# dusk-network/plonk

Measured on AMD Instinct MI355X. Metric: prove() wall-clock (ms) at 2^20 gates, lower is better.
Workload: dtype u32 limbs (Fr 256-bit / Fp 384-bit Montgomery)

## Files before the change

### plonk_amd/csrc/capi.hip

```cpp
#include <chrono>
#include <cstdio>
#include <cstring>
#include <sched.h>
#include <thread>

#include "plonk_internal.hpp"
#include "hostg1.hpp"

namespace plonk {

static thread_local char g_last_error[512] = "";

void set_last_error(const char* what, const char* detail, const char* file, int line) {
  snprintf(g_last_error, sizeof g_last_error, "%s:%d: %s -> %s", file, line, what ? what : "?", detail ? detail : "?");
}

int srs_generate_device(Ctx* c, const Fr& tau, const Fr& g_scalar, uint64_t n, G1Affine* out_dev);

int ctx_refuse_poisoned(const char* api_fn) {
  set_last_error(api_fn, "context unusable: a collective timed out and its stream never drained (comm_sync); destroy the context", __FILE__, __LINE__);
  return PLONK_ERR_STATE;
}

bool ctx_abandon(Ctx* c) {
  if (!c->comm_poisoned) return false;
  const auto t0 = std::chrono::steady_clock::now();
  for (;;) {
    const bool busy = (c->main_stream && hipStreamQuery(c->main_stream) == hipErrorNotReady) ||
                      (c->side_stream && hipStreamQuery(c->side_stream) == hipErrorNotReady);
    if (!busy) return false;
    if (std::chrono::duration_cast<std::chrono::milliseconds>(std::chrono::steady_clock::now() - t0).count() > 2000) return true;
    std::this_thread::sleep_for(std::chrono::microseconds(500));
  }
}

void xyzz_to_affine97_host(const G1& p, uint8_t out[97]) {
  G1Affine a;
  const bool finite = p.to_affine(&a);
  memcpy(out, a.x.l, 48);
  memcpy(out + 48, a.y.l, 48);
  out[96] = finite ? 0 : 1;
}

struct ProfRec { int slot; hipEvent_t a, b; };
struct ProfState {
  std::vector<hipEvent_t> pool;
  size_t used = 0;
  std::vector<ProfRec> recs;
  hipEvent_t open[Ctx::PROF_SLOTS] = {nullptr};
};
static std::map<Ctx*, ProfState*> g_prof;
static std::mutex g_prof_mu;

static ProfState* prof_state(Ctx* c) {
  std::lock_guard<std::mutex> lk(g_prof_mu);
  auto it = g_prof.find(c);
  if (it != g_prof.end()) return it->second;
  return g_prof[c] = new ProfState();
}
static void prof_release(Ctx* c) {
  ProfState* ps = nullptr;
  {
    std::lock_guard<std::mutex> lk(g_prof_mu);
    auto it = g_prof.find(c);
    if (it == g_prof.end()) return;
    ps = it->second;
    g_prof.erase(it);
  }
  for (hipEvent_t e : ps->pool) (void)hipEventDestroy(e);
  delete ps;
}
static void prof_forget(Ctx* c) {
  std::lock_guard<std::mutex> lk(g_prof_mu);
  auto it = g_prof.find(c);
  if (it != g_prof.end()) { delete it->second; g_prof.erase(it); }
}
static hipEvent_t prof_event(ProfState* ps) {
  if (ps->used == ps->pool.size()) {
    hipEvent_t e;
    if (hipEventCreate(&e) != hipSuccess) return nullptr;
    ps->pool.push_back(e);
  }
  return ps->pool[ps->used++];
}
void prof_begin(Ctx* c, int slot) {
  if (!c->profile) return;
  ProfState* ps = prof_state(c);
  hipEvent_t e = prof_event(ps);
  if (!e) return;
  (void)hipEventRecord(e, c->stream);
  ps->open[slot] = e;
}
void prof_end(Ctx* c, int slot) {
  if (!c->profile) return;
  ProfState* ps = prof_state(c);
  if (!ps->open[slot]) return;
  hipEvent_t e = prof_event(ps);
  if (!e) return;
  (void)hipEventRecord(e, c->stream);
  ps->recs.push_back({slot, ps->open[slot], e});
  ps->open[slot] = nullptr;
}
void prof_host_add(Ctx* c, int slot, double ms) {
  if (!c->profile) return;
  c->acc_ms[slot] += ms;
  c->acc_n[slot] += 1;
}
static int prof_collect(Ctx* c) {
  ProfState* ps = prof_state(c);
  HIP_TRY(hipStreamSynchronize(c->stream));
  for (auto& r : ps->recs) {
    float ms = 0;
    if (hipEventElapsedTime(&ms, r.a, r.b) == hipSuccess) {
      c->acc_ms[r.slot] += ms;
      c->acc_n[r.slot] += 1;
    }
  }
  ps->recs.clear();
  ps->used = 0;
  return PLONK_OK;
}

static int ensure_ntt_staging(Ctx* c, uint64_t n) {
  if (n <= c->ntt_cap) return PLONK_OK;
  if (c->ntt_buf) {
    HIP_TRY(hipStreamSynchronize(c->stream));
    HIP_TRY(hipFree(c->ntt_buf)); HIP_TRY(hipFree(c->ntt_buf2)); HIP_TRY(hipFree(c->ntt_buf3)); HIP_TRY(hipFree(c->ntt_tmp));
    c->ntt_buf = c->ntt_buf2 = c->ntt_buf3 = c->ntt_tmp = nullptr; c->ntt_cap = 0;
  }
  HIP_TRY(hipMalloc((void**)&c->ntt_buf, sizeof(Fr) * n));
  HIP_TRY(hipMalloc((void**)&c->ntt_buf2, sizeof(Fr) * n));
  HIP_TRY(hipMalloc((void**)&c->ntt_buf3, sizeof(Fr) * n));
  HIP_TRY(hipMalloc((void**)&c->ntt_tmp, sizeof(Fr) * n));
  c->ntt_cap = n;
  return PLONK_OK;
}

int msm_group_sums(Ctx* c, const Fr* const* scalars_dev, const uint64_t* m, int cnt, G1* sums) {
  G1* res[MSM_MAX_BATCH];
  for (int k = 0; k < cnt; ++k) res[k] = (G1*)c->msm.result + (size_t)k * MSM_BIT_SUMS;
  const int rc = msm_batch_device(c, scalars_dev, m, cnt, res, true);
  if (rc) return rc;
  HIP_TRY(hipMemcpyAsync(c->msm.result_host, c->msm.result, sizeof(G1) * MSM_BIT_SUMS * cnt, hipMemcpyDeviceToHost, c->stream));
  HIP_TRY(hipStreamSynchronize(c->stream));
  for (int k = 0; k < cnt; ++k)
    sums[k] = finish_bit_sums(reinterpret_cast<const G1*>(c->msm.result_host) + (size_t)k * MSM_BIT_SUMS, c->msm.last_rowbits,
                              c->srs_rows == MSM_ROWS_BITPOS);
  return PLONK_OK;
}

static int ensure_scalar_staging(Ctx* c, uint64_t m) {
  MsmWork& w = c->msm;
  if (m <= w.cap_stage) return PLONK_OK;
  if (w.scalars_stage) { HIP_TRY(hipFree(w.scalars_stage)); w.scalars_stage = nullptr; w.cap_stage = 0; }
  HIP_TRY(hipMalloc((void**)&w.scalars_stage, sizeof(Fr) * m));
  w.cap_stage = m;
  return PLONK_OK;
}

}

using namespace plonk;

namespace plonk {

static int env_int(const char* name, int dflt) { const char* e = getenv(name); return e && e[0] ? atoi(e) : dflt; }
static char env_chr(const char* name) { const char* e = getenv(name); return e ? e[0] : 0; }

void config_resolve(const plonk_gpu_config* user, int device, Config* out) {
  Config g;
  plonk_gpu_config u{};
  if (user) memcpy(&u, user, user->struct_size < sizeof(u) ? user->struct_size : sizeof(u));
  g.table_budget = u.table_budget_bytes;
  g.table_mode = u.table_mode;
  g.bucket_bits = u.msm_bucket_bits;
  g.quotient_domain = u.quotient_domain == 8 ? 8 : 4;
  g.wire_commit_coeff = u.wire_commit == 1;
  g.shard_quotient = u.shard_quotient;
  g.shard_z = u.shard_grand_product;
  g.shard_side = u.shard_side_stream;
  g.ntt_elog = u.ntt_elements_log2;
  g.comm_timeout_ms = u.comm_timeout_ms > 0 ? u.comm_timeout_ms : 120000;
  g.side_cus = u.side_stream_cus;
  switch (env_chr("PLONK_MSM_TABLE")) { case 'w': g.table_mode = MSM_ROWS_WINDOW; break; case 'h': g.table_mode = MSM_ROWS_HALFPOS; break; case 'b': g.table_mode = MSM_ROWS_BITPOS; break; default: break; }
  if (const int mb = env_int("PLONK_TABLE_BUDGET_MB", 0); mb > 0) g.table_budget = (uint64_t)mb << 20;
  if (const int b = env_int("PLONK_MSM_BUCKETS", 0); b) g.bucket_bits = b;
  if (env_chr("PLONK_QUOTIENT_DOMAIN") == '8') g.quotient_domain = 8;
  if (env_chr("PLONK_QUOTIENT_DOMAIN") == '4') g.quotient_domain = 4;
  if (env_chr("PLONK_WIRE_COMMIT") == 'c') g.wire_commit_coeff = 1;
  if (env_chr("PLONK_Z_COMMIT") == 'c') g.z_commit_coeff = 1;
  if (env_chr("PLONK_Z_COMMIT") == 'e') g.z_commit_coeff = -1;
  if (const char v = env_chr("PLONK_SHARD_QUOTIENT")) g.shard_quotient = v == '0' ? -1 : 1;
  if (const char v = env_chr("PLONK_SHARD_Z")) g.shard_z = v == '1' ? 1 : -1;
  if (const char v = env_chr("PLONK_SHARD_SIDE")) g.shard_side = v == '0' ? -1 : 1;
  if (const char v = env_chr("PLONK_NTT_ELOG"); v == '2' || v == '3') g.ntt_elog = v - '0';
  if (const int t = env_int("PLONK_COMM_TIMEOUT_MS", 0); t > 0) g.comm_timeout_ms = t;
  if (getenv("PLONK_SIDE_CUS")) g.side_cus = env_int("PLONK_SIDE_CUS", 0);
  g.ksl = env_int("PLONK_MSM_KSL", 0);
  g.prof_fine = env_chr("PLONK_PROF_FINE") == '1';
  g.acc_lds = env_chr("PLONK_MSM_ACC") == 'l';
  if (const char v = env_chr("PLONK_MSM_ORDER")) g.order = v == '1' ? 1 : 0;
  g.tail_serial = env_chr("PLONK_MSM_TAIL") == 's';
  g.bsum_lane = env_chr("PLONK_MSM_BSUM") == 'l';
  g.rc_lane_tree = env_chr("PLONK_MSM_RCTREE") == 'l';
  g.lps = env_int("PLONK_MSM_LPS", 0);
  g.rcwv = env_int("PLONK_MSM_RCWV", 0);
  if (const char v = env_chr("PLONK_MSM_SORT13")) g.sort13 = v == '1' ? 1 : 0;
  g.acc_wg = env_int("PLONK_MSM_ACC_WG", 0);
  g.ntt_direct = env_chr("PLONK_NTT_DIRECT") != '0';
  g.bi_cfg = env_int("PLONK_BI_CFG", -1);
  if (const char v = env_chr("PLONK_SIDE_DEFER")) g.side_defer = v == '1' ? 1 : (v == '2' ? 2 : 0);
  if (const char v = env_chr("PLONK_SIDE_AFTER_ELOG"); v == '2' || v == '3') g.side_after_elog = v - '0';
  if (const char v = env_chr("PLONK_WIRE_POLYS_SIDE")) g.wire_polys_side = v == '1' ? 1 : 0;
  if (env_chr("PLONK_WIRE_BY_COLUMN") == '0') g.wire_by_column = -1;
  if (env_chr("PLONK_WIRE_BY_COLUMN") == '1') g.wire_by_column = 1;
  if (env_chr("PLONK_WIRE_BY_COLUMN") == '2') g.wire_by_column = 2;
  if (getenv("PLONK_HOST_THREADS")) g.host_threads = env_int("PLONK_HOST_THREADS", -1);
  if (g.table_mode != (int)MSM_ROWS_WINDOW && g.table_mode != (int)MSM_ROWS_HALFPOS && g.table_mode != (int)MSM_ROWS_BITPOS) g.table_mode = 0;
  if (g.ntt_elog != 2 && g.ntt_elog != 3) g.ntt_elog = 0;
  if (g.side_cus < 0) g.side_cus = 0;
  if (g.host_threads < 0) {
    cpu_set_t set;
    CPU_ZERO(&set);
    const int cpus = sched_getaffinity(0, sizeof set, &set) == 0 ? CPU_COUNT(&set) : (int)std::thread::hardware_concurrency();
    g.host_threads = cpus >= 8 ? 3 : 0;
  }
  if (g.host_threads > 7) g.host_threads = 7;
  if (g.table_budget == 0) {
    size_t total = 0;
    if (hipDeviceTotalMem(&total, device) != hipSuccess || total == 0) total = 256ull << 30;
    g.table_budget = (uint64_t)total / 10 * 8;
  }
  *out = g;
}

static int config_check(const plonk_gpu_config* u, const char* api_fn) {
  if (!u) return PLONK_OK;
  if (u->struct_size < 8 || u->struct_size > 4096) return (set_last_error("invalid argument", "plonk_gpu_config.struct_size is not set", __FILE__, __LINE__), PLONK_ERR_ARG);
  plonk_gpu_config c{};
  memcpy(&c, u, u->struct_size < sizeof(c) ? u->struct_size : sizeof(c));
  auto bad = [&](const char* what) { set_last_error(api_fn, what, __FILE__, __LINE__); return PLONK_ERR_ARG; };
  if (c.table_mode != PLONK_TABLE_AUTO && c.table_mode != PLONK_TABLE_WINDOW && c.table_mode != PLONK_TABLE_HALFPOS && c.table_mode != PLONK_TABLE_BITPOS) return bad("plonk_gpu_config.table_mode");
  if (c.msm_bucket_bits != 0 && c.msm_bucket_bits != 15 && c.msm_bucket_bits != 17 && c.msm_bucket_bits != 19) return bad("plonk_gpu_config.msm_bucket_bits");
  if (c.quotient_domain != 0 && c.quotient_domain != 4 && c.quotient_domain != 8) return bad("plonk_gpu_config.quotient_domain");
  if (c.wire_commit != 0 && c.wire_commit != 1) return bad("plonk_gpu_config.wire_commit");
  if (c.ntt_elements_log2 != 0 && c.ntt_elements_log2 != 2 && c.ntt_elements_log2 != 3) return bad("plonk_gpu_config.ntt_elements_log2");
  for (int v : {c.shard_quotient, c.shard_grand_product, c.shard_side_stream}) if (v < -1 || v > 1) return bad("plonk_gpu_config.shard_*: -1, 0 or 1");
  if (c.comm_timeout_ms < 0 || c.side_stream_cus < -1 || c.side_stream_cus > 200) return bad("plonk_gpu_config.comm_timeout_ms / side_stream_cus");
  return PLONK_OK;
}

static int side_stream_partition(Ctx* c) {
  const int k = c->cfg.side_cus;
  if (k <= 0) return PLONK_OK;
  hipDeviceProp_t prop;
  HIP_TRY(hipGetDeviceProperties(&prop, c->device));
  const int ncu = prop.multiProcessorCount;
  if (k >= ncu) return (set_last_error("plonk_gpu_config.side_stream_cus", "must be smaller than the device's compute-unit count", __FILE__, __LINE__), PLONK_ERR_ARG);
  const int words = (ncu + 31) / 32;
  std::vector<uint32_t> side(words, 0u);
  for (int i = 0; i < ncu; ++i)
    if ((int64_t)i * k / ncu != (int64_t)(i + 1) * k / ncu) side[i / 32] |= 1u << (i % 32);
  hipStream_t ss = nullptr;
  if (hipExtStreamCreateWithCUMask(&ss, (uint32_t)words, side.data()) != hipSuccess) return (set_last_error("hipExtStreamCreateWithCUMask", "side stream", __FILE__, __LINE__), PLONK_ERR_HIP);
  (void)hipStreamDestroy(c->side_stream);
  c->side_stream = ss;
  return PLONK_OK;
}

}

extern "C" {

const char* plonk_last_error(void) { return g_last_error; }

static int create_context(plonk_ctx** out, int dev, const plonk_gpu_config* config, const char* api_fn) {
  if (!out) return PLONK_ERR_ARG;
  { const int rc = config_check(config, api_fn); if (rc) return rc; }
  int count = 0;
  if (hipGetDeviceCount(&count) != hipSuccess || count == 0) {
    set_last_error("hipGetDeviceCount", "no HIP device visible", __FILE__, __LINE__);
    return PLONK_ERR_NO_GPU;
  }
  if (dev < 0 || dev >= count) return PLONK_ERR_ARG;
  HIP_TRY(hipSetDevice(dev));
  auto* ctx = new plonk_ctx();
  ctx->c.device = dev;
  config_resolve(config, dev, &ctx->c.cfg);
  int prio_least = 0, prio_greatest = 0;
  (void)hipDeviceGetStreamPriorityRange(&prio_least, &prio_greatest);
  hipError_t e = hipStreamCreateWithPriority(&ctx->c.stream, hipStreamNonBlocking, prio_greatest);
  if (e == hipSuccess) e = hipStreamCreateWithPriority(&ctx->c.side_stream, hipStreamNonBlocking, prio_least);
  ctx->c.main_stream = ctx->c.stream;
  if (e != hipSuccess) {
    set_last_error("hipStreamCreate", hipGetErrorString(e), __FILE__, __LINE__);
    delete ctx;
    return PLONK_ERR_HIP;
  }
  { const int rc = side_stream_partition(&ctx->c); if (rc) { (void)hipStreamDestroy(ctx->c.stream); (void)hipStreamDestroy(ctx->c.side_stream); delete ctx; return rc; } }
  *out = ctx;
  return PLONK_OK;
}

int plonk_ctx_create(plonk_ctx** out, const int* devices, int ndev) {
  const char* const api_fn = __func__;
  return plonk::api_guard(api_fn, [&]() -> int {
  if (!out || ndev > 1 || ndev < 0) return PLONK_ERR_ARG;
  return create_context(out, (devices && ndev == 1) ? devices[0] : 0, nullptr, api_fn);
  });
}

int plonk_ctx_create_ex(plonk_ctx** out, int device, const plonk_gpu_config* config) {
  const char* const api_fn = __func__;
  return plonk::api_guard(api_fn, [&]() -> int { return create_context(out, device, config, api_fn); });
}

int plonk_ctx_get_config(plonk_ctx* ctx, plonk_gpu_config* out) {
  const char* const api_fn = __func__;
  return plonk::api_guard(api_fn, [&]() -> int {
  if (!ctx || !out || out->struct_size < 8 || out->struct_size > 4096) return (set_last_error("invalid argument", "plonk_ctx_get_config: set struct_size = sizeof(plonk_gpu_config)", __FILE__, __LINE__), PLONK_ERR_ARG);
  std::lock_guard<std::mutex> lk(ctx->c.mu);
  const Config& g = ctx->c.cfg;
  plonk_gpu_config full{};
  full.struct_size = (uint32_t)sizeof(plonk_gpu_config);
  full.table_budget_bytes = g.table_budget;
  full.table_mode = g.table_mode;
  full.msm_bucket_bits = g.bucket_bits;
  full.quotient_domain = g.quotient_domain;
  full.wire_commit = g.wire_commit_coeff;
  full.shard_quotient = g.shard_quotient;
  full.shard_grand_product = g.shard_z;
  full.shard_side_stream = g.shard_side;
  full.ntt_elements_log2 = g.ntt_elog;
  full.comm_timeout_ms = g.comm_timeout_ms;
  full.side_stream_cus = g.side_cus;
  const uint32_t want = out->struct_size < sizeof(full) ? out->struct_size : (uint32_t)sizeof(full);
  memcpy(out, &full, want);
  out->struct_size = want;
  return PLONK_OK;
  });
}

int plonk_ctx_set_config(plonk_ctx* ctx, const plonk_gpu_config* config) {
  const char* const api_fn = __func__;
  return plonk::api_guard(api_fn, [&]() -> int {
  if (!ctx) return PLONK_ERR_ARG;
  { const int rc = config_check(config, api_fn); if (rc) return rc; }
  std::lock_guard<std::mutex> lk(ctx->c.mu);
  Config next;
  config_resolve(config, ctx->c.device, &next);
  if (next.side_cus != ctx->c.cfg.side_cus)
    return (set_last_error("plonk_ctx_set_config", "side_stream_cus can only be chosen at plonk_ctx_create_ex", __FILE__, __LINE__), PLONK_ERR_STATE);
  ctx->c.cfg = next;
  return PLONK_OK;
  });
}

int plonk_ctx_table_bytes(plonk_ctx* ctx, uint64_t* in_use, uint64_t* budget) {
  const char* const api_fn = __func__;
  return plonk::api_guard(api_fn, [&]() -> int {
  if (!ctx) return PLONK_ERR_ARG;
  std::lock_guard<std::mutex> lk(ctx->c.mu);
  if (in_use) *in_use = ctx->c.table_bytes;
  if (budget) *budget = ctx->c.cfg.table_budget;
  return PLONK_OK;
  });
}

static void plan_out(const plonk_msm_plan_internal& p, plonk_msm_plan* out) {
  memset(out, 0, sizeof(*out));
  out->table_rows = p.table_rows; out->bucket_bits = p.bucket_bits; out->digit_width = p.digit_width;
  out->slice_entries = p.slice_entries; out->ordered_lanes = p.ordered_lanes; out->wide_words = p.wide_words; out->flags = p.flags; out->terms = p.terms;
  snprintf(out->accumulate_kernel, sizeof(out->accumulate_kernel), "%s", p.kernel);
}

int plonk_ctx_describe_msm(plonk_ctx* ctx, uint64_t m, int count, int bit_sum_tail, uint32_t table_rows, uint64_t table_points, plonk_msm_plan* out) {
  const char* const api_fn = __func__;
  return plonk::api_guard(api_fn, [&]() -> int {
  if (!ctx || !out || count < 1 || count > MSM_MAX_BATCH) return PLONK_ERR_ARG;
  std::lock_guard<std::mutex> lk(ctx->c.mu);
  Ctx& c = ctx->c;
  if (table_rows == 0) { table_rows = c.srs_rows; table_points = c.srs_n; if (!c.srs_table) return PLONK_ERR_NO_SRS; }
  if (table_rows != MSM_ROWS_WINDOW && table_rows != MSM_ROWS_HALFPOS && table_rows != MSM_ROWS_BITPOS) return PLONK_ERR_ARG;
  plonk_msm_plan_internal p;
  msm_plan(&c, table_rows, table_points, m, count, bit_sum_tail != 0, &p);
  plan_out(p, out);
  return PLONK_OK;
  });
}

int plonk_ctx_last_msm(plonk_ctx* ctx, plonk_msm_plan* out) {
  const char* const api_fn = __func__;
  return plonk::api_guard(api_fn, [&]() -> int {
  if (!ctx || !out) return PLONK_ERR_ARG;
  std::lock_guard<std::mutex> lk(ctx->c.mu);
  if (!ctx->c.last_plan.table_rows) return (set_last_error("plonk_ctx_last_msm", "no MSM has run on this context", __FILE__, __LINE__), PLONK_ERR_STATE);
  plan_out(ctx->c.last_plan, out);
  return PLONK_OK;
  });
}

void plonk_ctx_destroy(plonk_ctx* ctx) {
  if (!ctx) return;
  (void)plonk_comm_destroy(ctx);
  Ctx& c = ctx->c;
  finish_pool_release(&c);
  (void)hipSetDevice(c.device);
  if (ctx_abandon(&c)) {
    prof_forget(&c);
    delete ctx;
    return;
  }
  (void)hipStreamSynchronize(c.stream);
  verify_ws_release(&c);
  kzg_ws_release(&c);
  for (auto& kv : c.ntt_tables) {
    NttTables* t = kv.second;
    (void)hipFree(t->tw_lo); (void)hipFree(t->tw_hi); (void)hipFree(t->tw_lo_scaled);
    (void)hipFree(t->w512); (void)hipFree(t->g_lo); (void)hipFree(t->g_hi);
    (void)hipFree(t->tw_lo29); (void)hipFree(t->tw_hi29); (void)hipFree(t->tw_lo_scaled29);
    (void)hipFree(t->w512_29); (void)hipFree(t->g_lo29); (void)hipFree(t->g_hi29);
    (void)hipFree(t->tw_a29); (void)hipFree(t->tw_b29);
    delete t;
  }
  (void)hipFree(c.ntt_buf); (void)hipFree(c.ntt_buf2); (void)hipFree(c.ntt_buf3); (void)hipFree(c.ntt_tmp);
  if (c.down_stream) (void)hipStreamDestroy(c.down_stream);
  if (c.copy_stream) (void)hipStreamDestroy(c.copy_stream); (void)hipFree(c.srs_table); (void)hipFree(c.table_scratch);
  MsmWork& w = c.msm;
  (void)hipFree(w.tmp_words); (void)hipFree(w.entries); (void)hipFree(w.coarse_cnt); (void)hipFree(w.coarse_off); (void)hipFree(w.coarse_cur); (void)hipFree(w.big_off); (void)hipFree(w.big_cnt); (void)hipFree(w.nheavy); (void)hipFree(w.heavy_list); (void)hipFree(w.seg_sum);
  (void)hipFree(w.offsets); (void)hipFree(w.slice_off); (void)hipFree(w.full_off); (void)hipFree(w.part_list); (void)hipFree(w.partial); (void)hipFree(w.buckets);
  (void)hipFree(w.multi_list); (void)hipFree(w.layout);
  (void)hipFree(w.chunk); (void)hipFree(w.result); (void)hipFree(w.scalars_stage);
  if (w.result_host) (void)hipHostFree(w.result_host);
  prof_release(&c);
  (void)hipStreamDestroy(c.main_stream);
  if (c.side_stream) (void)hipStreamDestroy(c.side_stream);
  delete ctx;
}

int plonk_ctx_table_rows(plonk_ctx* ctx) { return ctx ? (int)ctx->c.srs_rows : 0; }
void* plonk_ctx_stream(plonk_ctx* ctx) { return ctx ? (void*)ctx->c.main_stream : nullptr; }

int plonk_dev_alloc(plonk_ctx* ctx, uint64_t bytes, void** out) {
  const char* const api_fn = __func__;
  return plonk::api_guard(api_fn, [&]() -> int {
  if (!ctx || !out) return PLONK_ERR_ARG;
  HIP_TRY(hipSetDevice(ctx->c.device));
  HIP_TRY(hipMalloc(out, bytes ? bytes : 1));
  return PLONK_OK;
  });
}
int plonk_dev_free(plonk_ctx* ctx, void* p) {
  const char* const api_fn = __func__;
  return plonk::api_guard(api_fn, [&]() -> int {
  if (!ctx) return PLONK_ERR_ARG;
  CTX_ENTER(ctx->c, api_fn);
  HIP_TRY(hipSetDevice(ctx->c.device));
  HIP_TRY(hipStreamSynchronize(ctx->c.main_stream));
  HIP_TRY(hipFree(p));
  return PLONK_OK;
  });
}
int plonk_dev_h2d(plonk_ctx* ctx, void* dst, const void* src, uint64_t bytes) {
  const char* const api_fn = __func__;
  return plonk::api_guard(api_fn, [&]() -> int {
  if (!ctx || (!dst && bytes) || (!src && bytes)) return PLONK_ERR_ARG;
  CTX_ENTER(ctx->c, api_fn);
  HIP_TRY(hipSetDevice(ctx->c.device));
  HIP_TRY(hipMemcpyAsync(dst, src, bytes, hipMemcpyHostToDevice, ctx->c.main_stream));
  HIP_TRY(hipStreamSynchronize(ctx->c.main_stream));
  return PLONK_OK;
  });
}
int plonk_dev_d2h(plonk_ctx* ctx, void* dst, const void* src, uint64_t bytes) {
  const char* const api_fn = __func__;
  return plonk::api_guard(api_fn, [&]() -> int {
  if (!ctx || (!dst && bytes) || (!src && bytes)) return PLONK_ERR_ARG;
  CTX_ENTER(ctx->c, api_fn);
  HIP_TRY(hipSetDevice(ctx->c.device));
  HIP_TRY(hipMemcpyAsync(dst, src, bytes, hipMemcpyDeviceToHost, ctx->c.main_stream));
  HIP_TRY(hipStreamSynchronize(ctx->c.main_stream));
  return PLONK_OK;
  });
}
int plonk_dev_sync(plonk_ctx* ctx) {
  const char* const api_fn = __func__;
  return plonk::api_guard(api_fn, [&]() -> int {
  if (!ctx) return PLONK_ERR_ARG;
  CTX_ENTER(ctx->c, api_fn);
  HIP_TRY(hipSetDevice(ctx->c.device));
  HIP_TRY(hipStreamSynchronize(ctx->c.main_stream));
  return PLONK_OK;
  });
}

int plonk_ntt_dev(plonk_ctx* ctx, const void* src, void* dst, void* tmp, uint32_t log_n, int inverse,
                  int coset, uint64_t in_len) {
  const char* const api_fn = __func__;
  return plonk::api_guard(api_fn, [&]() -> int {
  if (!ctx || !src || !dst || log_n >= 28) return PLONK_ERR_ARG;
  if (log_n > 10 && !tmp) return PLONK_ERR_ARG;
  CTX_ENTER(ctx->c, api_fn);
  HIP_TRY(hipSetDevice(ctx->c.device));
  prof_begin(&ctx->c, 0);
  int rc = ntt_device(&ctx->c, (const Fr*)src, (Fr*)dst, (Fr*)tmp, log_n, inverse != 0, coset != 0, in_len);
  prof_end(&ctx->c, 0);
  return rc;
  });
}

int plonk_ntt(plonk_ctx* ctx, uint64_t* a, uint32_t log_n, int inverse, int coset, uint64_t in_len) {
  const char* const api_fn = __func__;
  return plonk::api_guard(api_fn, [&]() -> int {
  if (!ctx || !a || log_n >= 28) return PLONK_ERR_ARG;
  Ctx& c = ctx->c;
  CTX_ENTER(c, api_fn);
  HIP_TRY(hipSetDevice(c.device));
  const uint64_t n = 1ull << log_n;
  if (in_len > n) in_len = n;
  int rc = ensure_ntt_staging(&c, n);
  if (rc) return rc;
  HIP_TRY(hipMemcpyAsync(c.ntt_buf, a, sizeof(Fr) * in_len, hipMemcpyHostToDevice, c.stream));
  rc = ntt_device(&c, c.ntt_buf, c.ntt_buf, c.ntt_tmp, log_n, inverse != 0, coset != 0, in_len);
  if (rc) return rc;
  HIP_TRY(hipMemcpyAsync(a, c.ntt_buf, sizeof(Fr) * n, hipMemcpyDeviceToHost, c.stream));
  HIP_TRY(hipStreamSynchronize(c.stream));
  return PLONK_OK;
  });
}

int plonk_ntt_batch(plonk_ctx* ctx, uint64_t* const* a, int count, uint32_t log_n, int inverse, int coset,
                    const uint64_t* in_len) {
  const char* const api_fn = __func__;
  return plonk::api_guard(api_fn, [&]() -> int {
  if (!ctx || !a || count < 0 || log_n >= 28) return PLONK_ERR_ARG;
  for (int i = 0; i < count; ++i) if (!a[i]) return PLONK_ERR_ARG;
  if (count == 0) return PLONK_OK;
  Ctx& c = ctx->c;
  CTX_ENTER(c, api_fn);
  HIP_TRY(hipSetDevice(c.device));
  const uint64_t n = 1ull << log_n;
  int rc = ensure_ntt_staging(&c, n);
  if (rc) return rc;
  if (!c.copy_stream) HIP_TRY(hipStreamCreateWithFlags(&c.copy_stream, hipStreamNonBlocking));
  if (!c.down_stream) HIP_TRY(hipStreamCreateWithFlags(&c.down_stream, hipStreamNonBlocking));
  Fr* buf[3] = {c.ntt_buf, c.ntt_buf2, c.ntt_buf3};
  hipEvent_t up[3] = {nullptr, nullptr, nullptr}, done[3] = {nullptr, nullptr, nullptr}, freed[3] = {nullptr, nullptr, nullptr};
  hipError_t e = hipSuccess;
  for (int k = 0; k < 3 && e == hipSuccess; ++k) {
    e = hipEventCreateWithFlags(&up[k], hipEventDisableTiming);
    if (e == hipSuccess) e = hipEventCreateWithFlags(&done[k], hipEventDisableTiming);
    if (e == hipSuccess) e = hipEventCreateWithFlags(&freed[k], hipEventDisableTiming);
  }
  for (int k = 0; k < count && e == hipSuccess && rc == PLONK_OK; ++k) {
    const int b = k % 3;
    uint64_t len = in_len ? in_len[k] : n;
    if (len > n) len = n;
    if (k >= 3) e = hipStreamWaitEvent(c.copy_stream, freed[b], 0);
    if (e == hipSuccess) e = hipMemcpyAsync(buf[b], a[k], sizeof(Fr) * len, hipMemcpyHostToDevice, c.copy_stream);
    if (e == hipSuccess) e = hipEventRecord(up[b], c.copy_stream);
    if (e == hipSuccess) e = hipStreamWaitEvent(c.stream, up[b], 0);
    if (e == hipSuccess) rc = ntt_device(&c, buf[b], buf[b], c.ntt_tmp, log_n, inverse != 0, coset != 0, len);
    if (e == hipSuccess && rc == PLONK_OK) e = hipEventRecord(done[b], c.stream);
    if (e == hipSuccess && rc == PLONK_OK) e = hipStreamWaitEvent(c.down_stream, done[b], 0);
    if (e == hipSuccess && rc == PLONK_OK) e = hipMemcpyAsync(a[k], buf[b], sizeof(Fr) * n, hipMemcpyDeviceToHost, c.down_stream);
    if (e == hipSuccess && rc == PLONK_OK) e = hipEventRecord(freed[b], c.down_stream);
  }
  const hipError_t e1 = hipStreamSynchronize(c.copy_stream), e2 = hipStreamSynchronize(c.stream), e3 = hipStreamSynchronize(c.down_stream);
  if (e == hipSuccess) e = e1 != hipSuccess ? e1 : (e2 != hipSuccess ? e2 : e3);
  for (int k = 0; k < 3; ++k) {
    if (up[k]) (void)hipEventDestroy(up[k]);
    if (done[k]) (void)hipEventDestroy(done[k]);
    if (freed[k]) (void)hipEventDestroy(freed[k]);
  }
  if (e != hipSuccess) { set_last_error("plonk_ntt_batch", hipGetErrorString(e), __FILE__, __LINE__); if (rc == PLONK_OK) rc = PLONK_ERR_HIP; }
  return rc;
  });
}

int plonk_srs_load_dev(plonk_ctx* ctx, const void* xy96_dev, uint64_t npoints) {
  const char* const api_fn = __func__;
  return plonk::api_guard(api_fn, [&]() -> int {
  if (!ctx || (!xy96_dev && npoints)) return PLONK_ERR_ARG;
  CTX_ENTER(ctx->c, api_fn);
  HIP_TRY(hipSetDevice(ctx->c.device));
  return srs_load_device(&ctx->c, (const G1Affine*)xy96_dev, npoints);
  });
}

// ... 231 lines not shown
```

### plonk_amd/csrc/msm_sort.hip

```cpp
#include "plonk_internal.hpp"
#include "fr29.cuh"

namespace plonk {
namespace PLONK_MSM_NS {

static constexpr uint32_t FINE_BITS = MSM_NB_BITS - 11;
static constexpr uint32_t COARSE = MSM_NB >> FINE_BITS;
#ifndef PLONK_SORT_TILE
#define PLONK_SORT_TILE 2048
#endif
static constexpr uint32_t TILE = PLONK_SORT_TILE;
static constexpr uint32_t SORT_T = 1024;
static constexpr uint32_t PER_T = TILE / SORT_T;
#ifndef PLONK_HIST_PER
#define PLONK_HIST_PER 2
#endif
static constexpr uint32_t HIST_PER = PLONK_HIST_PER;
static constexpr uint32_t HIST_TILE = SORT_T * HIST_PER;
static_assert(COARSE == 2 * SORT_T, "scan / reservation loops assume two coarse bins per thread");
static constexpr uint32_t IDX_BITS = 31 - FINE_BITS;
static constexpr uint32_t IDX_MASK = (1u << IDX_BITS) - 1;
static_assert(IDX_BITS + 1 + FINE_BITS == 32, "narrow intermediate word layout");
template <class WordT> struct SortWord;
template <> struct SortWord<uint32_t> {
// ... 554 lines not shown
    if (t == 0) {
      uint32_t acc = 0;
      for (uint32_t r = ksl - 1; r >= 1; --r) { const uint32_t h = hist[r]; hist[r] = acc; acc += h; }
      hist[0] = acc;
    }
    __syncthreads();
    for (uint32_t i = t; i < MSM_NB; i += SORT_T) full_off[i] = stage[stage_at(i)];
    if (t == SORT_T - 1) full_off[MSM_NB] = total_f;
#pragma unroll
    for (uint32_t k = 0; k < PER; ++k) {
      const uint32_t r = (o[k + 1] - o[k]) & (ksl - 1);
      if (r) part_list[atomicAdd(&hist[r], 1u)] = t * PER + k;
    }
    if (t == 0) part_list[MSM_NB] = hist[0];
  }
}
#if PLONK_MSM_NB_BITS > 15
static constexpr uint32_t LAY_NBLK = MSM_NB / SORT_T, LAY_H = 132;
static constexpr uint32_t LAY_WORDS = 2 * LAY_NBLK + (LAY_NBLK + 1) * LAY_H;
__global__ void __launch_bounds__(SORT_T) msm_layout_count_kernel(const uint32_t* __restrict__ offsets_all, uint32_t* __restrict__ slice_off_all,
                                                                  uint32_t* __restrict__ full_off_all, uint32_t* __restrict__ lay_all, uint32_t ksl, int kb0) {
  __shared__ uint32_t sh[SORT_T];
  __shared__ uint32_t hist[LAY_H];
  const int kb = (int)blockIdx.y + kb0;
  const uint32_t blk = blockIdx.x, t = threadIdx.x, b = blk * SORT_T + t;
  const uint32_t* __restrict__ offsets = offsets_all + (uint64_t)kb * (MSM_NB + 1);
  uint32_t* __restrict__ lay = lay_all + (uint64_t)kb * LAY_WORDS;
  if (t < LAY_H) hist[t] = 0;
  __syncthreads();
  const uint32_t cnt = offsets[b + 1] - offsets[b];
  const uint32_t nf = cnt / ksl, r = cnt % ksl, ns = nf + (r ? 1u : 0u);
  if (r) atomicAdd(&hist[r], 1u);
  uint32_t tot_ns, tot_nf;
  const uint32_t ex_ns = block_exclusive_scan(ns, sh, &tot_ns);
  const uint32_t ex_nf = block_exclusive_scan(nf, sh, &tot_nf);
  slice_off_all[(uint64_t)kb * (MSM_NB + 1) + b] = ex_ns;
  full_off_all[(uint64_t)kb * (MSM_NB + 1) + b] = ex_nf;
  if (t == 0) { lay[blk] = tot_ns; lay[LAY_NBLK + blk] = tot_nf; }
  if (t < LAY_H) lay[2 * LAY_NBLK + blk * LAY_H + t] = hist[t];
}
__global__ void __launch_bounds__(SORT_T) msm_layout_scan_kernel(uint32_t* __restrict__ slice_off_all, uint32_t* __restrict__ full_off_all,
                                                                 uint32_t* __restrict__ part_list_all, uint32_t* __restrict__ lay_all, uint32_t ksl, int kb0) {
  __shared__ uint32_t sh[SORT_T];
  __shared__ uint32_t ctot[LAY_H];
  const int kb = (blockIdx.x + (uint32_t)kb0);
  const uint32_t t = threadIdx.x;
  uint32_t* __restrict__ lay = lay_all + (uint64_t)kb * LAY_WORDS;
  static_assert(LAY_NBLK <= SORT_T, "one thread per block total");
  uint32_t tot;
  const uint32_t a = t < LAY_NBLK ? lay[t] : 0u;
  const uint32_t ea = block_exclusive_scan(a, sh, &tot);
  if (t < LAY_NBLK) lay[t] = ea;
  if (t == 0) slice_off_all[(uint64_t)kb * (MSM_NB + 1) + MSM_NB] = tot;
  const uint32_t f = t < LAY_NBLK ? lay[LAY_NBLK + t] : 0u;
  const uint32_t ef = block_exclusive_scan(f, sh, &tot);
  if (t < LAY_NBLK) lay[LAY_NBLK + t] = ef;
  if (t == 0) full_off_all[(uint64_t)kb * (MSM_NB + 1) + MSM_NB] = tot;
  if (t < LAY_H) {
    uint32_t run = 0;
    if (t >= 1 && t < ksl)
      for (uint32_t blk = 0; blk < LAY_NBLK; ++blk) {
        uint32_t* q = lay + 2 * LAY_NBLK + blk * LAY_H + t;
        const uint32_t h = *q;
        *q = run;
        run += h;
      }
    ctot[t] = run;
  }
  __syncthreads();
  if (t == 0) {
    uint32_t acc = 0;
    uint32_t* cstart = lay + 2 * LAY_NBLK + LAY_NBLK * LAY_H;
    for (uint32_t r = ksl - 1; r >= 1; --r) { cstart[r] = acc; acc += ctot[r]; }
    part_list_all[(uint64_t)kb * (MSM_NB + 1) + MSM_NB] = acc;
  }
}
__global__ void __launch_bounds__(SORT_T) msm_layout_apply_kernel(const uint32_t* __restrict__ offsets_all, uint32_t* __restrict__ slice_off_all,
                                                                  uint32_t* __restrict__ full_off_all, uint32_t* __restrict__ part_list_all,
                                                                  const uint32_t* __restrict__ lay_all, uint32_t ksl, uint32_t heavy_thresh,
                                                                  uint32_t* __restrict__ nheavy_all, HeavyItem* __restrict__ heavy_list_all,
                                                                  uint4* __restrict__ buckets_raw, uint32_t* __restrict__ multi_list_all, int kb0) {
  __shared__ uint32_t rank[LAY_H];
  const int kb = (int)blockIdx.y + kb0;
  const uint32_t blk = blockIdx.x, t = threadIdx.x, b = blk * SORT_T + t;
  const uint32_t* __restrict__ offsets = offsets_all + (uint64_t)kb * (MSM_NB + 1);
  const uint32_t* __restrict__ lay = lay_all + (uint64_t)kb * LAY_WORDS;
  if (t < LAY_H) rank[t] = 0;
  __syncthreads();
  const uint32_t cnt = offsets[b + 1] - offsets[b];
  const uint32_t nf = cnt / ksl, r = cnt % ksl, ns = nf + (r ? 1u : 0u);
  slice_off_all[(uint64_t)kb * (MSM_NB + 1) + b] += lay[blk];
  full_off_all[(uint64_t)kb * (MSM_NB + 1) + b] += lay[LAY_NBLK + blk];
  if (r) {
    const uint32_t pos = lay[2 * LAY_NBLK + LAY_NBLK * LAY_H + r] + lay[2 * LAY_NBLK + blk * LAY_H + r] + atomicAdd(&rank[r], 1u);
    part_list_all[(uint64_t)kb * (MSM_NB + 1) + pos] = b;
  }
  if (ns > heavy_thresh) {
    HeavyItem it;
    it.bucket = b;
    it.nseg = (ns + HEAVY_SEG_SLICES - 1) / HEAVY_SEG_SLICES;
    it.seg_base = atomicAdd(&nheavy_all[2 * kb + 1], it.nseg);
    it.pad = 0;
    heavy_list_all[(uint64_t)kb * MSM_NB + atomicAdd(&nheavy_all[2 * kb], 1u)] = it;
  } else if (ns == 0) {
    uint4* q = buckets_raw + ((uint64_t)kb * MSM_NB + b) * 16;
#pragma unroll
    for (int k = 0; k < 16; ++k) q[k] = make_uint4(0u, 0u, 0u, 0u);
  }
  __shared__ uint32_t nmul, mbase;
  if (t == 0) nmul = 0;
  __syncthreads();
  const bool multi = ns >= 2 && ns <= heavy_thresh;
  const uint32_t mrank = multi ? atomicAdd(&nmul, 1u) : 0u;
  __syncthreads();
  if (t == 0 && nmul) mbase = atomicAdd(&nheavy_all[2 * MSM_MAX_BATCH + kb], nmul);
  __syncthreads();
  if (multi) multi_list_all[(uint64_t)kb * MSM_NB + mbase + mrank] = b;
}
#endif

int msm_order_slices(Ctx* c, const MsmBatch& bt) {
  (void)c; (void)bt;
  return PLONK_OK;
}

template <int MODE, class WordT>
static int msm_group_sort_t(Ctx* c, const MsmBatch& bt, uint64_t mmax) {
  MsmWork& w = c->msm;
  hipStream_t st = c->stream;
  const uint32_t tiles = (uint32_t)((mmax + TILE - 1) / TILE);
  const uint32_t htiles = (uint32_t)((mmax + HIST_TILE - 1) / HIST_TILE);
  void* tmp = (void*)w.tmp_words;
  const int kb0 = bt.kb0;
  HIP_TRY(hipMemsetAsync(w.coarse_cnt + (size_t)COARSE * kb0, 0, sizeof(uint32_t) * COARSE * bt.count, st));
  hipLaunchKernelGGL(msm_hist_kernel<MODE>, dim3(htiles, bt.count), dim3(SORT_T), 0, st, bt, w.coarse_cnt);
  hipLaunchKernelGGL(msm_coarse_scan_kernel, dim3(bt.count), dim3(SORT_T), 0, st, w.coarse_cnt, w.coarse_off, w.coarse_cur, w.big_off, kb0);
#if PLONK_MSM_NB_BITS >= 19
  if constexpr (MODE != 0) {
    if (c->cfg.sort13 == 1) {
      const uint32_t tiles2 = (uint32_t)((mmax + P2_TILE - 1) / P2_TILE);
      smem_opt_in(c, (const void*)msm_partition2_kernel<MODE, WordT>, PARTITION2_LDS);
      hipLaunchKernelGGL((msm_partition2_kernel<MODE, WordT>), dim3(tiles2, bt.count), dim3(P2_T), PARTITION2_LDS, st, bt, bt.table_n,
                         w.coarse_off, w.coarse_cur, tmp);
    }
  }
  if (MODE == 0 || c->cfg.sort13 != 1) {
#else
  {
#endif
    smem_opt_in(c, (const void*)msm_partition_kernel<MODE, WordT>, PARTITION_LDS);
    hipLaunchKernelGGL((msm_partition_kernel<MODE, WordT>), dim3(tiles, bt.count), dim3(SORT_T), PARTITION_LDS, st, bt, bt.table_n,
                       w.coarse_off, w.coarse_cur, tmp);
  }
  hipLaunchKernelGGL(msm_fine_kernel<WordT>, dim3(COARSE, bt.count), dim3(FINE_T), 0, st, bt, w.coarse_off, tmp,
                     w.entries, w.offsets);
  {
    const uint64_t words = (uint64_t)MSM_W * mmax;
    const uint32_t most = (uint32_t)(words / BIG_CHUNK + words / BIG_LIMIT + 1);
    const uint32_t big_wgs = most < 512u ? most : 512u;
    if (kb0 == 0 && bt.count == bt.group_count) {
      HIP_TRY(hipMemsetAsync(w.big_cnt, 0, sizeof(uint32_t) * 2 * MSM_NB * MSM_MAX_BATCH, st));
    } else {
      HIP_TRY(hipMemsetAsync(w.big_cnt + (size_t)MSM_NB * kb0, 0, sizeof(uint32_t) * MSM_NB * bt.count, st));
      HIP_TRY(hipMemsetAsync(w.big_cnt + (size_t)MSM_NB * MSM_MAX_BATCH + (size_t)MSM_NB * kb0, 0, sizeof(uint32_t) * MSM_NB * bt.count, st));
    }
    hipLaunchKernelGGL(msm_big_hist_kernel<WordT>, dim3(big_wgs, bt.count), dim3(BIG_T), 0, st, bt, w.coarse_off, w.big_off, tmp, w.big_cnt);
    hipLaunchKernelGGL(msm_big_scatter_kernel<WordT>, dim3(big_wgs, bt.count), dim3(BIG_T), 0, st, bt, w.coarse_off, w.big_off, tmp,
                       w.big_cnt, w.big_cnt + (size_t)MSM_NB * MSM_MAX_BATCH, w.entries, w.offsets);
  }
  if (kb0 == 0 && bt.count == bt.group_count) {
    HIP_TRY(hipMemsetAsync(w.nheavy, 0, sizeof(uint32_t) * 4 * MSM_MAX_BATCH, st));
  } else {
    HIP_TRY(hipMemsetAsync(w.nheavy + 2 * kb0, 0, sizeof(uint32_t) * 2 * bt.count, st));
    HIP_TRY(hipMemsetAsync(w.nheavy + 2 * MSM_MAX_BATCH + kb0, 0, sizeof(uint32_t) * bt.count, st));
  }
#if PLONK_MSM_NB_BITS > 15
  if (bt.ksl > 128) return (set_last_error("msm_group_sort", "slice length above 128", __FILE__, __LINE__), PLONK_ERR_ARG);
  hipLaunchKernelGGL(msm_layout_count_kernel, dim3(LAY_NBLK, bt.count), dim3(SORT_T), 0, st, w.offsets, w.slice_off, w.full_off, w.layout, bt.ksl, kb0);
  hipLaunchKernelGGL(msm_layout_scan_kernel, dim3(bt.count), dim3(SORT_T), 0, st, w.slice_off, w.full_off, w.part_list, w.layout, bt.ksl, kb0);
  hipLaunchKernelGGL(msm_layout_apply_kernel, dim3(LAY_NBLK, bt.count), dim3(SORT_T), 0, st, w.offsets, w.slice_off, w.full_off, w.part_list,
                     (const uint32_t*)w.layout, bt.ksl, bt.heavy_thresh, w.nheavy, (HeavyItem*)w.heavy_list, (uint4*)w.buckets, w.multi_list, kb0);
#else
  if (bt.ordered) {
    if (bt.ksl > 128) return (set_last_error("msm_group_sort", "slice length above 128", __FILE__, __LINE__), PLONK_ERR_ARG);
    smem_opt_in(c, (const void*)msm_slices_kernel<true>, SLICES_LDS);
    hipLaunchKernelGGL(msm_slices_kernel<true>, dim3(bt.count), dim3(SORT_T), SLICES_LDS, st, w.offsets, w.slice_off, bt.ksl, bt.heavy_thresh,
                       w.nheavy, (HeavyItem*)w.heavy_list, kb0, w.full_off, w.part_list);
  } else {
    smem_opt_in(c, (const void*)msm_slices_kernel<false>, SLICES_LDS);
    hipLaunchKernelGGL(msm_slices_kernel<false>, dim3(bt.count), dim3(SORT_T), SLICES_LDS, st, w.offsets, w.slice_off, bt.ksl, bt.heavy_thresh,
                       w.nheavy, (HeavyItem*)w.heavy_list, kb0, (uint32_t*)nullptr, (uint32_t*)nullptr);
  }
#endif
  HIP_TRY(hipGetLastError());
  return PLONK_OK;
}
int msm_group_sort(Ctx* c, const MsmBatch& bt, uint64_t mmax) {
  if ((uint64_t)bt.rows * bt.table_n > (1ull << 31))
    return (set_last_error("commit key too large for the bucket sort", "table rows * points must be <= 2^31", __FILE__, __LINE__), PLONK_ERR_ARG);
  if (bt.rows == MSM_ROWS_BITPOS) return bt.wide ? msm_group_sort_t<1, uint64_t>(c, bt, mmax) : msm_group_sort_t<1, uint32_t>(c, bt, mmax);
  if (bt.rows == MSM_ROWS_HALFPOS) return bt.wide ? msm_group_sort_t<2, uint64_t>(c, bt, mmax) : msm_group_sort_t<2, uint32_t>(c, bt, mmax);
#if PLONK_MSM_NB_BITS == 15
  return bt.wide ? msm_group_sort_t<0, uint64_t>(c, bt, mmax) : msm_group_sort_t<0, uint32_t>(c, bt, mmax);
#else
  return (set_last_error("msm_group_sort", "window tables need the 2^15-bucket variant", __FILE__, __LINE__), PLONK_ERR_ARG);
#endif
}
bool msm_needs_wide_words(uint32_t rows, uint64_t table_n) { return (uint64_t)rows * table_n > (1ull << IDX_BITS); }

}
}
```

### plonk_amd/csrc/plonk_internal.hpp

```cpp
#pragma once
#include <hip/hip_runtime.h>
#include <stdint.h>

#include <map>
#include <mutex>
#include <set>
#include <vector>

#include "../../include/plonk_hip.h"
#include "api_guard.hpp"
#include "curve.cuh"
#include "msm_recode.cuh"

#define HIP_TRY(expr)                                                    \
  do {                                                                   \
    hipError_t _e = (expr);                                              \
    if (_e != hipSuccess) {                                              \
      plonk::set_last_error(#expr, hipGetErrorString(_e), __FILE__, __LINE__); \
      return PLONK_ERR_HIP;                                              \
    }                                                                    \
  } while (0)

namespace plonk {

void set_last_error(const char* what, const char* detail, const char* file, int line);
struct Ctx;
int ctx_refuse_poisoned(const char* api_fn);
void finish_pool_release(Ctx* c);
void verify_ws_release(Ctx* c);
bool ctx_abandon(Ctx* c);
#define CTX_ENTER(C, FN)                      \
  std::lock_guard<std::mutex> lk((C).mu);     \
  if ((C).comm_poisoned) return plonk::ctx_refuse_poisoned(FN)

struct NttTables {
  Fr* tw_lo = nullptr;
  Fr* tw_hi = nullptr;
  Fr* tw_lo_scaled = nullptr;
  Fr* w512 = nullptr;
  Fr* g_lo = nullptr;
  Fr* g_hi = nullptr;
  void* tw_lo29 = nullptr;
  void* tw_hi29 = nullptr;
  void* tw_lo_scaled29 = nullptr;
  void* w512_29 = nullptr;
  void* g_lo29 = nullptr;
  void* g_hi29 = nullptr;
  void* tw_a29 = nullptr;
  void* tw_b29 = nullptr;
  Fr n_inv;
};

#ifndef PLONK_MSM_NB_BITS
#define PLONK_MSM_NB_BITS 15
#endif
#if PLONK_MSM_NB_BITS == 15
#define PLONK_MSM_NS nb15
#elif PLONK_MSM_NB_BITS == 17
#define PLONK_MSM_NS nbm
#elif PLONK_MSM_NB_BITS >= 18 && PLONK_MSM_NB_BITS <= 19
#define PLONK_MSM_NS nbl
#else
#error "PLONK_MSM_NB_BITS must be 15 or 17..19"
#endif
static constexpr int MSM_C = 16;
static constexpr int MSM_W = MSM_DIGITS;
static constexpr int MSM_NB_BITS = PLONK_MSM_NB_BITS;
static constexpr uint32_t MSM_NB = 1u << MSM_NB_BITS;
static constexpr int MSM_NB_BITS_MAX = 19;
static constexpr uint32_t MSM_NB_MAX = 1u << MSM_NB_BITS_MAX;
static constexpr uint32_t MSM_NAF_WIDTH = MSM_NB_BITS + 2;
static constexpr int MSM_MAX_BATCH = 4;

struct MsmBatch {
  const Fr* scalars[MSM_MAX_BATCH];
  uint64_t m[MSM_MAX_BATCH];
  G1* out[MSM_MAX_BATCH];
  int count;
  uint32_t ksl;
  uint64_t cap_m, cap_slices;
  const void* table;
  uint64_t table_n;
  uint32_t rows;
  uint32_t ordered;
  uint32_t wide;
  uint32_t heavy_thresh;
  const Fr* tail[MSM_MAX_BATCH];
  uint64_t split[MSM_MAX_BATCH];
  int kb0;
  int group_count;
};

struct HeavyItem { uint32_t bucket, seg_base, nseg, pad; };

struct MsmWork {
  bool fixed_ok = false;
  uint64_t cap_m = 0;
  uint32_t* tmp_words = nullptr;
  uint32_t* entries = nullptr;
  uint32_t* coarse_cnt = nullptr;
  uint32_t* coarse_off = nullptr;
  uint32_t* coarse_cur = nullptr;
  uint32_t* big_off = nullptr;
  uint32_t* big_cnt = nullptr;
  uint32_t* offsets = nullptr;
  uint32_t* slice_off = nullptr;
  uint32_t* full_off = nullptr;
  uint32_t* part_list = nullptr;
  uint32_t* multi_list = nullptr;
  uint32_t* layout = nullptr;
  uint64_t cap_slices = 0;
  void* partial = nullptr;
  void* buckets = nullptr;
  uint32_t* nheavy = nullptr;
  void* heavy_list = nullptr;
  void* seg_sum = nullptr;
  uint64_t cap_segs = 0;
  void* chunk = nullptr;
  int last_rowbits = 8;
  uint8_t* result = nullptr;
  uint8_t* result_host = nullptr;
  Fr* scalars_stage = nullptr;
  uint64_t cap_stage = 0;
};

struct Config {
  uint64_t table_budget = 0;
  int table_mode = 0;
  int bucket_bits = 0;
  int quotient_domain = 4;
  int wire_commit_coeff = 0;
  int z_commit_coeff = 0;
  int shard_quotient = 0;
  int shard_z = 0;
  int shard_side = 0;
  int ntt_elog = 0;
  int comm_timeout_ms = 120000;
  int side_cus = 0;
  int ksl = 0;
  bool prof_fine = false;
  bool acc_lds = false;
  int order = -1;
  bool tail_serial = false;
  bool bsum_lane = false;
  bool rc_lane_tree = false;
  int lps = 0;
  int rcwv = 0;
  int sort13 = -1;
  int acc_wg = 0;
  bool ntt_direct = true;
  int bi_cfg = -1;
  int side_defer = -1;
  int wire_by_column = 0;
  int wire_polys_side = -1;
  int side_after_elog = 0;
  int host_threads = -1;
};

struct plonk_msm_plan_internal {
  uint32_t table_rows = 0, bucket_bits = 0, digit_width = 0, slice_entries = 0, ordered_lanes = 0, wide_words = 0, flags = 0;
  uint64_t terms = 0;
  const char* kernel = "";
};

struct Ctx {
  int device = 0;
  Config cfg;
  uint64_t srs_table_alloc = 0;
  uint64_t table_bytes = 0;
  plonk_msm_plan_internal last_plan;
  hipStream_t stream = nullptr;
  hipStream_t main_stream = nullptr;
  hipStream_t side_stream = nullptr;
  hipEvent_t acc_done = nullptr;
  int ntt_elog_hint = 0;
  std::mutex mu;
  std::mutex table_mu;
  std::map<uint32_t, NttTables*> ntt_tables;
  std::set<const void*> smem_opt_in;
  Fr* ntt_buf = nullptr;
  Fr* ntt_buf2 = nullptr;
  Fr* ntt_buf3 = nullptr;
  hipStream_t copy_stream = nullptr;
  hipStream_t down_stream = nullptr;
  Fr* ntt_tmp = nullptr;
  uint64_t ntt_cap = 0;
  void* srs_table = nullptr;
  uint32_t srs_rows = 0;
  void* table_scratch = nullptr;
  uint64_t table_scratch_pts = 0;
  uint64_t srs_n = 0;
  uint64_t srs_gen = 0;
  MsmWork msm;
  void* nccl_comm = nullptr;
  uint8_t* comm_send = nullptr;
  uint8_t* comm_recv = nullptr;
  uint8_t* comm_send_host = nullptr;
  uint8_t* comm_recv_host = nullptr;
  int comm_rank = 0, comm_world = 1;
  const char* comm_warning = "";
  bool comm_poisoned = false;
  bool comm_loopback = false;
  void* finish_pool = nullptr;
  void* verify_ws = nullptr;
  void* kzg_ws = nullptr;
  bool profile = false;
  hipEvent_t ev0 = nullptr, ev1 = nullptr;
  static constexpr int PROF_SLOTS = 32;
  double acc_ms[PROF_SLOTS] = {0};
  uint64_t acc_n[PROF_SLOTS] = {0};
};

struct NttCoset {
  Fr* g_lo = nullptr;
  Fr* g_hi = nullptr;
  void* g_lo29 = nullptr;
  void* g_hi29 = nullptr;
};
int ntt_coset_tables(Ctx* c, uint32_t L, const Fr& shift, bool inverse, NttCoset* out);
void ntt_coset_free(NttCoset* t);
int ntt_device(Ctx* c, const Fr* src, Fr* dst, Fr* tmp, uint32_t L, bool inverse, bool coset, uint64_t in_len,
               const NttCoset* shift = nullptr);
int ntt_tables(Ctx* c, uint32_t L, bool inverse, NttTables** out);
inline void smem_opt_in(Ctx* c, const void* fn, size_t bytes) {
  if (c->smem_opt_in.insert(fn).second) (void)hipFuncSetAttribute(fn, hipFuncAttributeMaxDynamicSharedMemorySize, (int)bytes);
}
void ntt_plan(uint32_t L, int r[3], int* npass);

struct CommLink {
  int rank = 0, world = 1;
  plonk_allgather_fn fn = nullptr;
  void* user = nullptr;
};
int comm_allgather_host(Ctx* c, const CommLink& l, const void* send, void* recv, size_t bytes);
int comm_sync(Ctx* c, hipStream_t st);
int comm_alltoall_dev(Ctx* c, const CommLink& l, const void* send_dev, void* recv_dev, size_t bytes_per_peer);
int comm_allgather_dev(Ctx* c, const CommLink& l, void* buf_dev, size_t bytes_per_rank);

int srs_load_device(Ctx* c, const G1Affine* pts_dev, uint64_t n);
int srs_table_begin(Ctx* c, uint64_t n);
int srs_table_chunk(Ctx* c, const G1Affine* pts_dev, uint64_t n, uint64_t first, uint64_t count, hipStream_t st);
void srs_table_scratch_free(Ctx* c);
int srs_validate_device(Ctx* c, const G1Affine* pts_dev, uint64_t n, int* flag_dev);
int srs_export_device(Ctx* c, G1Affine* out_dev);
int msm_device(Ctx* c, const Fr* scalars_dev, uint64_t m, G1* out_xyzz_dev);
static constexpr int MSM_BIT_SUMS = 12 + 9;
#define PLONK_MSM_VARIANT_DECLS                                                                                          \
  int msm_order_slices(Ctx* c, const MsmBatch& bt);                                                                      \
  int msm_group_sort(Ctx* c, const MsmBatch& bt, uint64_t mmax);                                                         \
  bool msm_needs_wide_words(uint32_t rows, uint64_t table_n);                                                            \
  int msm_batch_device_v(Ctx* c, MsmBatch& bt, uint64_t mmax, bool bit_sums, int phase);                                 \
  uint32_t msm_ksl(const Ctx* c, uint64_t m);                                                                            \
  bool msm_acc_ordered(const Ctx* c, uint32_t ksl);
namespace nb15 { PLONK_MSM_VARIANT_DECLS }
#ifdef PLONK_MSM_WITH_MEDIUM
namespace nbm { PLONK_MSM_VARIANT_DECLS int msm_buckets_bits(); }
#endif
namespace nbl { PLONK_MSM_VARIANT_DECLS int msm_buckets_bits(); }
int msm_batch_device(Ctx* c, const Fr* const* scalars_dev, const uint64_t* m, int count, G1* const* out_xyzz_dev,
                     bool bit_sums = false, const void* table = nullptr, uint64_t table_n = 0,
                     const Fr* const* tail_dev = nullptr, const uint64_t* split = nullptr, uint32_t table_rows = 0,
                     int phase = 3, int kb0 = 0, int kcount = -1);
uint32_t msm_table_rows(const Ctx* c, uint64_t n, bool last_key);
uint64_t msm_table_bytes(uint32_t rows, uint64_t n);
void msm_plan(const Ctx* c, uint32_t table_rows, uint64_t table_n, uint64_t mmax, int count, bool bit_sums, plonk_msm_plan_internal* out);
void config_resolve(const plonk_gpu_config* user, int device, Config* out);
int srs_table_build(Ctx* c, const G1Affine* pts_dev, uint64_t n, void** table_out, uint32_t* rows_out);
void srs_table_release(Ctx* c, void* table, uint32_t rows, uint64_t n);
int lagrange_points_device(Ctx* c, uint32_t L, G1Affine* out_dev);
int lagrange_blind_points_device(Ctx* c, uint64_t n, uint32_t k0, uint32_t cnt, G1Affine* out_dev);
int xyzz_to_affine97_device(Ctx* c, const G1* in_dev, uint8_t* out97_dev);
void xyzz_to_affine97_host(const G1& p, uint8_t out[97]);
int msm_reserve(Ctx* c, uint64_t m);

struct H1;
struct G1Aff64;
struct G2Prepared;
enum : int { VDEC_OK = 0, VDEC_IDENTITY = 1, VDEC_BAD = 2 };
static constexpr uint32_t VERIFY_MSM_MAX_BLOCKS = 512;
int decode_points(Ctx* c, const uint8_t* comp_host, uint32_t n, uint8_t* comp_dev, G1Affine* pts_dev, int32_t* kind_dev,
                  std::vector<int32_t>* st);
int msm_run(Ctx* c, const uint32_t* sc, const uint32_t* ids, uint64_t nL, uint64_t nR, const G1Affine* pts,
            const int32_t* kind, G1* part_dev, H1 sums[2]);
bool pairing_check(const H1 sums[2], const G2Prepared& x_h, const G2Prepared& h);
G1Aff64 xyzz_to_aff(const H1& p);
int msm_group_sums(Ctx* c, const Fr* const* scalars_dev, const uint64_t* m, int cnt, G1* sums);
void kzg_ws_release(Ctx* c);
int msm_sort_reserve_fixed(Ctx* c);

}

struct plonk_ctx {
  plonk::Ctx c;
};
```

Measured before the change: 30.95.

## Overlap MSM big-bucket sort kernels with fine sort on an auxiliary stream

Result: no change. 30.99 (+0.1%).

```diff
diff --git a/plonk_amd/csrc/capi.hip b/plonk_amd/csrc/capi.hip
--- a/plonk_amd/csrc/capi.hip
+++ b/plonk_amd/csrc/capi.hip
@@ -27,11 +27,32 @@
   const auto t0 = std::chrono::steady_clock::now();
   for (;;) {
     const bool busy = (c->main_stream && hipStreamQuery(c->main_stream) == hipErrorNotReady) ||
-                      (c->side_stream && hipStreamQuery(c->side_stream) == hipErrorNotReady);
+                      (c->side_stream && hipStreamQuery(c->side_stream) == hipErrorNotReady) ||
+                      (c->aux_stream && hipStreamQuery(c->aux_stream) == hipErrorNotReady);
     if (!busy) return false;
     if (std::chrono::duration_cast<std::chrono::milliseconds>(std::chrono::steady_clock::now() - t0).count() > 2000) return true;
     std::this_thread::sleep_for(std::chrono::microseconds(500));
   }
+}
+
+int aux_stream_get(Ctx* c) {
+  if (c->aux_stream) return PLONK_OK;
+  int prio_least = 0, prio_greatest = 0;
+  (void)hipDeviceGetStreamPriorityRange(&prio_least, &prio_greatest);
+  hipStream_t s = nullptr;
+  hipEvent_t f = nullptr, j = nullptr;
+  hipError_t e = hipStreamCreateWithPriority(&s, hipStreamNonBlocking, prio_greatest);
+  if (e == hipSuccess) e = hipEventCreateWithFlags(&f, hipEventDisableTiming);
+  if (e == hipSuccess) e = hipEventCreateWithFlags(&j, hipEventDisableTiming);
+  if (e != hipSuccess) {
+    if (j) (void)hipEventDestroy(j);
+    if (f) (void)hipEventDestroy(f);
+    if (s) (void)hipStreamDestroy(s);
+    set_last_error("auxiliary stream", hipGetErrorString(e), __FILE__, __LINE__);
+    return PLONK_ERR_HIP;
+  }
+  c->aux_stream = s; c->aux_fork = f; c->aux_join = j;
+  return PLONK_OK;
 }
 
 void xyzz_to_affine97_host(const G1& p, uint8_t out[97]) {
@@ -212,6 +233,7 @@
   if (const char v = env_chr("PLONK_SIDE_DEFER")) g.side_defer = v == '1' ? 1 : (v == '2' ? 2 : 0);
   if (const char v = env_chr("PLONK_SIDE_AFTER_ELOG"); v == '2' || v == '3') g.side_after_elog = v - '0';
   if (const char v = env_chr("PLONK_WIRE_POLYS_SIDE")) g.wire_polys_side = v == '1' ? 1 : 0;
+  if (const char v = env_chr("PLONK_MSM_OVERLAP")) g.msm_overlap = v == '0' ? 0 : 1;
   if (env_chr("PLONK_WIRE_BY_COLUMN") == '0') g.wire_by_column = -1;
   if (env_chr("PLONK_WIRE_BY_COLUMN") == '1') g.wire_by_column = 1;
   if (env_chr("PLONK_WIRE_BY_COLUMN") == '2') g.wire_by_column = 2;
@@ -435,6 +457,9 @@
   prof_release(&c);
   (void)hipStreamDestroy(c.main_stream);
   if (c.side_stream) (void)hipStreamDestroy(c.side_stream);
+  if (c.aux_stream) (void)hipStreamDestroy(c.aux_stream);
+  if (c.aux_fork) (void)hipEventDestroy(c.aux_fork);
+  if (c.aux_join) (void)hipEventDestroy(c.aux_join);
   delete ctx;
 }
 
diff --git a/plonk_amd/csrc/msm_sort.hip b/plonk_amd/csrc/msm_sort.hip
--- a/plonk_amd/csrc/msm_sort.hip
+++ b/plonk_amd/csrc/msm_sort.hip
@@ -730,6 +730,14 @@
     hipLaunchKernelGGL((msm_partition_kernel<MODE, WordT>), dim3(tiles, bt.count), dim3(SORT_T), PARTITION_LDS, st, bt, bt.table_n,
                        w.coarse_off, w.coarse_cur, tmp);
   }
+  hipStream_t bst = st;
+  if (c->cfg.msm_overlap) {
+    const int rc = aux_stream_get(c);
+    if (rc) return rc;
+    bst = c->aux_stream;
+    HIP_TRY(hipEventRecord(c->aux_fork, st));
+    HIP_TRY(hipStreamWaitEvent(bst, c->aux_fork, 0));
+  }
   hipLaunchKernelGGL(msm_fine_kernel<WordT>, dim3(COARSE, bt.count), dim3(FINE_T), 0, st, bt, w.coarse_off, tmp,
                      w.entries, w.offsets);
   {
@@ -737,14 +745,18 @@
     const uint32_t most = (uint32_t)(words / BIG_CHUNK + words / BIG_LIMIT + 1);
     const uint32_t big_wgs = most < 512u ? most : 512u;
     if (kb0 == 0 && bt.count == bt.group_count) {
-      HIP_TRY(hipMemsetAsync(w.big_cnt, 0, sizeof(uint32_t) * 2 * MSM_NB * MSM_MAX_BATCH, st));
+      HIP_TRY(hipMemsetAsync(w.big_cnt, 0, sizeof(uint32_t) * 2 * MSM_NB * MSM_MAX_BATCH, bst));
     } else {
-      HIP_TRY(hipMemsetAsync(w.big_cnt + (size_t)MSM_NB * kb0, 0, sizeof(uint32_t) * MSM_NB * bt.count, st));
-      HIP_TRY(hipMemsetAsync(w.big_cnt + (size_t)MSM_NB * MSM_MAX_BATCH + (size_t)MSM_NB * kb0, 0, sizeof(uint32_t) * MSM_NB * bt.count, st));
-    }
-    hipLaunchKernelGGL(msm_big_hist_kernel<WordT>, dim3(big_wgs, bt.count), dim3(BIG_T), 0, st, bt, w.coarse_off, w.big_off, tmp, w.big_cnt);
-    hipLaunchKernelGGL(msm_big_scatter_kernel<WordT>, dim3(big_wgs, bt.count), dim3(BIG_T), 0, st, bt, w.coarse_off, w.big_off, tmp,
+      HIP_TRY(hipMemsetAsync(w.big_cnt + (size_t)MSM_NB * kb0, 0, sizeof(uint32_t) * MSM_NB * bt.count, bst));
+      HIP_TRY(hipMemsetAsync(w.big_cnt + (size_t)MSM_NB * MSM_MAX_BATCH + (size_t)MSM_NB * kb0, 0, sizeof(uint32_t) * MSM_NB * bt.count, bst));
+    }
+    hipLaunchKernelGGL(msm_big_hist_kernel<WordT>, dim3(big_wgs, bt.count), dim3(BIG_T), 0, bst, bt, w.coarse_off, w.big_off, tmp, w.big_cnt);
+    hipLaunchKernelGGL(msm_big_scatter_kernel<WordT>, dim3(big_wgs, bt.count), dim3(BIG_T), 0, bst, bt, w.coarse_off, w.big_off, tmp,
                        w.big_cnt, w.big_cnt + (size_t)MSM_NB * MSM_MAX_BATCH, w.entries, w.offsets);
+  }
+  if (bst != st) {
+    HIP_TRY(hipEventRecord(c->aux_join, bst));
+    HIP_TRY(hipStreamWaitEvent(st, c->aux_join, 0));
   }
   if (kb0 == 0 && bt.count == bt.group_count) {
     HIP_TRY(hipMemsetAsync(w.nheavy, 0, sizeof(uint32_t) * 4 * MSM_MAX_BATCH, st));
diff --git a/plonk_amd/csrc/plonk_internal.hpp b/plonk_amd/csrc/plonk_internal.hpp
--- a/plonk_amd/csrc/plonk_internal.hpp
+++ b/plonk_amd/csrc/plonk_internal.hpp
@@ -154,6 +154,7 @@
   int wire_by_column = 0;
   int wire_polys_side = -1;
   int side_after_elog = 0;
+  int msm_overlap = 1;
   int host_threads = -1;
 };
 
@@ -172,6 +173,8 @@
   hipStream_t stream = nullptr;
   hipStream_t main_stream = nullptr;
   hipStream_t side_stream = nullptr;
+  hipStream_t aux_stream = nullptr;
+  hipEvent_t aux_fork = nullptr, aux_join = nullptr;
   hipEvent_t acc_done = nullptr;
   int ntt_elog_hint = 0;
   std::mutex mu;
@@ -226,6 +229,7 @@
   if (c->smem_opt_in.insert(fn).second) (void)hipFuncSetAttribute(fn, hipFuncAttributeMaxDynamicSharedMemorySize, (int)bytes);
 }
 void ntt_plan(uint32_t L, int r[3], int* npass);
+int aux_stream_get(Ctx* c);
 
 struct CommLink {
   int rank = 0, world = 1;
```
